# MengLing-L/distributed_plonk

Measured on AMD Instinct MI355X. Metric: constraints/sec = n / proof time (verified five-round proof, dispatcher2.rs:192-713; BN254 PLONK), higher is better.
Workload: dtype u32x8 Montgomery (256-bit Fr/Fq)

## Files before the change

### distributed_plonk_amd/csrc/msm_engine.hip

```cpp
#include <algorithm>
#include <cstring>

#include "constants.h"
#include "ec.hpp"
#include "ec_lazy.hpp"
#include "plonk_internal.hpp"

#define BASES_BAD_CURVE 1u
#define BASES_BAD_RANGE 2u
#define BASES_BAD_FLAG 4u
template <int NQ> static const FpParams<NQ>& fq_params(int curve);
template <> const FpParams<8>& fq_params<8>(int) { return BN254_FQ_PARAMS; }
template <> const FpParams<12>& fq_params<12>(int) { return BLS12_381_FQ_PARAMS; }

#ifndef MSM_SIDE_PRIO
#define MSM_SIDE_PRIO 0
#endif
#if MSM_SIDE_PRIO > 0
#define MSM_SIDE_PRIO_ENTER() __builtin_amdgcn_s_setprio(MSM_SIDE_PRIO)
#else
#define MSM_SIDE_PRIO_ENTER() ((void)0)
#endif

template <typename T> __device__ __forceinline__ T load16(const T* p) {
    static_assert(sizeof(T) % 16 == 0, "16-byte multiple");
    T r;
    const uint4* s = reinterpret_cast<const uint4*>(p);
    uint4* d = reinterpret_cast<uint4*>(&r);
#pragma unroll
    for (unsigned i = 0; i < sizeof(T) / 16; i++) d[i] = s[i];
    return r;
}
template <typename T> __device__ __forceinline__ void store16(T* p, const T& v) {
    uint4* d = reinterpret_cast<uint4*>(p);
    const uint4* s = reinterpret_cast<const uint4*>(&v);
#pragma unroll
    for (unsigned i = 0; i < sizeof(T) / 16; i++) d[i] = s[i];
}

__device__ __forceinline__ uint32_t scalar_raw_digit(const uint32_t* s, int bit0, int c) {
    const int limb = bit0 >> 5, off = bit0 & 31;
    if (limb >= 8) return 0;
    uint64_t v = s[limb];
    if (limb + 1 < 8) v |= (uint64_t)s[limb + 1] << 32;
    return (uint32_t)(v >> off) & ((1u << c) - 1);
}

__global__ void __launch_bounds__(256) msm_digits_kernel(const uint32_t* __restrict__ scalars, uint64_t n, uint64_t len, int c, int W,
                                                         uint32_t* __restrict__ dig, int scalars_mont, const FpParams<8> FR) {
    MSM_SIDE_PRIO_ENTER();
    const uint64_t i = (uint64_t)blockIdx.x * blockDim.x + threadIdx.x;
    if (i >= n) return;
    if (i >= len) {
        for (int w = 0; w < W; w++) dig[(uint64_t)w * n + i] = 0;
        return;
    }
    uint32_t s[8];
    const uint4* sp = reinterpret_cast<const uint4*>(scalars + 8 * i);
    const uint4 lo = sp[0], hi = sp[1];
    s[0] = lo.x; s[1] = lo.y; s[2] = lo.z; s[3] = lo.w; s[4] = hi.x; s[5] = hi.y; s[6] = hi.z; s[7] = hi.w;
    if (scalars_mont) {
        Fp<8> v;
#pragma unroll
        for (int k = 0; k < 8; k++) v.l[k] = s[k];
        v = fp_from_mont(v, FR);
#pragma unroll
        for (int k = 0; k < 8; k++) s[k] = v.l[k];
    }
    const uint32_t half = 1u << (c - 1);
    uint32_t carry = 0;
    for (int w = 0; w < W; w++) {
        const int bit0 = w * c, limb = bit0 >> 5, off = bit0 & 31;
        uint64_t v = 0;
#pragma unroll
        for (int k = 0; k < 8; k++) {
            if (k == limb) v |= s[k];
            if (k == limb + 1) v |= (uint64_t)s[k] << 32;
        }
        uint32_t raw = ((uint32_t)(v >> off) & ((1u << c) - 1)) + carry;
        carry = raw > half;
        const uint32_t mag = carry ? (1u << c) - raw : raw;
        dig[(uint64_t)w * n + i] = mag | (carry << 31);
    }
}

#define SORT_SLICE_LOG 14
#define SORT_SLICE (1 << SORT_SLICE_LOG)
struct SortGeom {
    uint64_t n;
    int W, cb, lp, low_bits;
    uint32_t nblk;
    uint32_t nreal;
    uint32_t idx_bits;
    uint32_t stage_cap;
};

__global__ void __launch_bounds__(256) sort_hist_kernel(const uint32_t* __restrict__ dig, SortGeom g, uint32_t* __restrict__ blk_hist) {
    MSM_SIDE_PRIO_ENTER();
    extern __shared__ uint32_t h[];
    const uint32_t np = (1u << g.lp) + 1;
    for (uint32_t k = threadIdx.x; k < np; k += blockDim.x) h[k] = 0;
    __syncthreads();
    const uint32_t w = blockIdx.y, blk = blockIdx.x;
    const uint64_t beg = (uint64_t)blk * SORT_SLICE, end = beg + SORT_SLICE < g.n ? beg + SORT_SLICE : g.n;
    const uint32_t* d = dig + (uint64_t)w * g.n;
    for (uint64_t i = beg + threadIdx.x; i < end; i += blockDim.x) {
        const uint32_t mag = d[i] & 0x7fffffffu;
        const uint32_t part = mag ? ((mag - 1) >> g.low_bits) : (np - 1);
        atomicAdd(&h[part], 1u);
    }
    __syncthreads();
    for (uint32_t k = threadIdx.x; k < np; k += blockDim.x) {
        const uint64_t pid = (k == np - 1) ? (uint64_t)g.nreal + w : ((uint64_t)w << g.lp) + k;
        blk_hist[pid * g.nblk + blk] = h[k];
    }
}

#define SCATTER_THREADS 1024
__global__ void __launch_bounds__(SCATTER_THREADS) sort_scatter_kernel(const uint32_t* __restrict__ dig, SortGeom g, const uint32_t* __restrict__ blk_off,
                                                                       uint32_t* __restrict__ tmp) {
    MSM_SIDE_PRIO_ENTER();
    extern __shared__ uint32_t sm[];
    const uint32_t np = (1u << g.lp) + 1;
    uint32_t* cnt = sm;
    uint32_t* loc = sm + np;
    uint32_t* buf = sm + 2 * np + 1;
    const uint32_t w = blockIdx.y, blk = blockIdx.x;
    for (uint32_t k = threadIdx.x; k < np; k += blockDim.x) cnt[k] = 0;
    __syncthreads();
    const uint64_t beg = (uint64_t)blk * SORT_SLICE, end = beg + SORT_SLICE < g.n ? beg + SORT_SLICE : g.n;
    const uint32_t* d = dig + (uint64_t)w * g.n;
    for (uint64_t i = beg + threadIdx.x; i < end; i += blockDim.x) {
        const uint32_t mag = d[i] & 0x7fffffffu;
        atomicAdd(&cnt[mag ? ((mag - 1) >> g.low_bits) : (np - 1)], 1u);
    }
    __syncthreads();
    __shared__ uint32_t strip[SCATTER_THREADS];
    const uint32_t per = (np + blockDim.x - 1) / blockDim.x;
    const uint32_t s0 = threadIdx.x * per < np ? threadIdx.x * per : np, s1 = s0 + per < np ? s0 + per : np;
    uint32_t acc = 0;
    for (uint32_t k = s0; k < s1; k++) acc += cnt[k];
    strip[threadIdx.x] = acc;
    __syncthreads();
    for (int dd = 1; dd < SCATTER_THREADS; dd <<= 1) {
        const uint32_t t = (int)threadIdx.x >= dd ? strip[threadIdx.x - dd] : 0;
        __syncthreads();
        strip[threadIdx.x] += t;
        __syncthreads();
    }
    uint32_t run = strip[threadIdx.x] - acc;
    for (uint32_t k = s0; k < s1; k++) { const uint32_t v = cnt[k]; loc[k] = run; cnt[k] = run; run += v; }
    if (threadIdx.x == blockDim.x - 1) loc[np] = strip[blockDim.x - 1];
    __syncthreads();
    const uint32_t low_mask = (1u << g.low_bits) - 1;
    const uint32_t ebits = (uint32_t)g.low_bits + SORT_SLICE_LOG + 1;
    const bool packed = ebits + (uint32_t)g.lp <= 32;
    for (uint64_t i = beg + threadIdx.x; i < end; i += blockDim.x) {
        const uint32_t e = d[i], mag = e & 0x7fffffffu;
        if (!mag) continue;
        const uint32_t key = mag - 1, part = key >> g.low_bits;
        const uint32_t pos = atomicAdd(&cnt[part], 1u);
        uint32_t v = ((key & low_mask) << (SORT_SLICE_LOG + 1)) | ((e >> 31) << SORT_SLICE_LOG) | (uint32_t)(i - beg);
        if (packed && g.lp) v |= part << ebits;
        buf[pos] = v;
    }
    __syncthreads();
    const uint32_t nreal_local = loc[np - 1];
    const uint32_t emask = ebits >= 32 ? 0xffffffffu : ((1u << ebits) - 1);
    for (uint32_t j = threadIdx.x; j < nreal_local; j += blockDim.x) {
        const uint32_t v = buf[j];
        uint32_t lo;
        if (packed) {
            lo = g.lp ? (v >> ebits) : 0;
        } else {
            lo = 0;
            uint32_t hi = np - 1;
            while (hi - lo > 1) { const uint32_t mid = (lo + hi) >> 1; if (loc[mid] <= j) lo = mid; else hi = mid; }
        }
        const uint64_t pid = ((uint64_t)w << g.lp) + lo;
        uint32_t out = packed ? (v & emask) : v;
        if (g.idx_bits) {
            const uint32_t in = out & (SORT_SLICE - 1), sg = (out >> SORT_SLICE_LOG) & 1u, lowb = out >> (SORT_SLICE_LOG + 1);
            out = (lowb << (g.idx_bits + 1)) | (sg << g.idx_bits) | (uint32_t)(beg + in);
        }
        tmp[blk_off[pid * g.nblk + blk] + (j - loc[lo])] = out;
    }
}

#define SIZE_BINS 256
struct SizeHist {
    uint32_t* ghist;
    uint32_t bin_shift;
    uint64_t nbuckets;
};
__device__ __forceinline__ uint32_t size_bin_of(uint32_t entries, uint32_t bin_shift) {
    const uint32_t sz = entries >> bin_shift;
    return (SIZE_BINS - 1) - (sz < SIZE_BINS - 1 ? sz : SIZE_BINS - 1);
}
__global__ void __launch_bounds__(256) sort_partition_kernel(const uint32_t* __restrict__ tmp, SortGeom g, const uint32_t* __restrict__ blk_off,
                                                             uint32_t* __restrict__ sorted, uint32_t* __restrict__ offsets, const SizeHist sz) {
    MSM_SIDE_PRIO_ENTER();
    extern __shared__ uint32_t lds[];
    __shared__ uint32_t shist[SIZE_BINS];
    if (sz.ghist) shist[threadIdx.x] = 0;
    const uint32_t nlow = 1u << g.low_bits;
    uint32_t* cnt = lds;
    uint32_t* run0 = lds + nlow;
    const uint64_t pid = blockIdx.x;
    const uint32_t* po = blk_off + pid * g.nblk;
    const uint32_t pbeg = po[0], pend = po[g.nblk];
    for (uint32_t k = threadIdx.x; k < nlow; k += blockDim.x) cnt[k] = 0;
    for (uint32_t k = threadIdx.x; k < g.nblk; k += blockDim.x) run0[k] = po[k];
    __syncthreads();
    const int sh = g.idx_bits ? (int)g.idx_bits + 1 : SORT_SLICE_LOG + 1;
    for (uint32_t j = pbeg + threadIdx.x; j < pend; j += blockDim.x) atomicAdd(&cnt[tmp[j] >> sh], 1u);
    __syncthreads();
    if (threadIdx.x == 0) {
        uint32_t run = pbeg;
        for (uint32_t k = 0; k < nlow; k++) {
            const uint32_t v = cnt[k];
            cnt[k] = run;
            run += v;
            if (sz.ghist && (pid << g.low_bits) + k < sz.nbuckets) shist[size_bin_of(v, sz.bin_shift)]++;
        }
    }
    __syncthreads();
    if (sz.ghist && shist[threadIdx.x]) atomicAdd(&sz.ghist[threadIdx.x], shist[threadIdx.x]);
    for (uint32_t k = threadIdx.x; k < nlow; k += blockDim.x) offsets[(pid << g.low_bits) + k] = cnt[k];
    if (pid == g.nreal - 1 && threadIdx.x == 0) offsets[(uint64_t)g.nreal << g.low_bits] = pend;
    __syncthreads();
    const uint32_t in_mask = SORT_SLICE - 1;
    if (g.idx_bits) {
        const uint32_t imask = (1u << g.idx_bits) - 1;
        for (uint32_t j = pbeg + threadIdx.x; j < pend; j += blockDim.x) {
            const uint32_t e = tmp[j];
            const uint32_t pos = atomicAdd(&cnt[e >> sh], 1u);
            sorted[pos] = (e & imask) | (((e >> g.idx_bits) & 1u) << 31);
        }
        return;
    }
    for (uint32_t j = pbeg + threadIdx.x; j < pend; j += blockDim.x) {
        const uint32_t e = tmp[j];
        uint32_t lo = 0, hi = g.nblk;
        while (hi - lo > 1) { const uint32_t mid = (lo + hi) >> 1; if (run0[mid] <= j) lo = mid; else hi = mid; }
        const uint32_t pos = atomicAdd(&cnt[e >> sh], 1u);
        sorted[pos] = ((lo << SORT_SLICE_LOG) + (e & in_mask)) | (((e >> SORT_SLICE_LOG) & 1u) << 31);
    }
}

#define STAGE_THREADS 1024
#define STAGE_MAX_CHUNKS 8u
__global__ void __launch_bounds__(STAGE_THREADS) sort_partition_staged_kernel(const uint32_t* __restrict__ tmp, SortGeom g, const uint32_t* __restrict__ blk_off,
                                                                              uint32_t* __restrict__ sorted, uint32_t* __restrict__ offsets, const SizeHist sz) {
    MSM_SIDE_PRIO_ENTER();
    extern __shared__ uint32_t lds[];
    __shared__ uint32_t shist[SIZE_BINS];
    if (sz.ghist && threadIdx.x < SIZE_BINS) shist[threadIdx.x] = 0;
    const uint32_t nlow = 1u << g.low_bits;
    uint32_t* cnt = lds;
    uint32_t* run0 = lds + nlow;
    uint32_t* buf = run0 + (g.idx_bits ? 0 : g.nblk);
    uint32_t* strip = buf;
    const uint64_t pid = blockIdx.x;
    const uint32_t* po = blk_off + pid * g.nblk;
    const uint32_t pbeg = po[0], pend = po[g.nblk], len = pend - pbeg;
    const int sh = g.idx_bits ? (int)g.idx_bits + 1 : SORT_SLICE_LOG + 1;
    for (uint32_t k = threadIdx.x; k < nlow; k += blockDim.x) cnt[k] = 0;
    if (!g.idx_bits)
        for (uint32_t k = threadIdx.x; k < g.nblk; k += blockDim.x) run0[k] = po[k];
    __syncthreads();
    for (uint32_t j = pbeg + threadIdx.x; j < pend; j += blockDim.x) atomicAdd(&cnt[tmp[j] >> sh], 1u);
    __syncthreads();
    const uint32_t per = (nlow + blockDim.x - 1) / blockDim.x;
    const uint32_t s0 = threadIdx.x * per < nlow ? threadIdx.x * per : nlow, s1 = s0 + per < nlow ? s0 + per : nlow;
    uint32_t acc = 0;
    for (uint32_t k = s0; k < s1; k++) acc += cnt[k];
    strip[threadIdx.x] = acc;
    __syncthreads();
    for (int dd = 1; dd < STAGE_THREADS; dd <<= 1) {
        const uint32_t t = (int)threadIdx.x >= dd ? strip[threadIdx.x - dd] : 0;
        __syncthreads();
        strip[threadIdx.x] += t;
        __syncthreads();
    }
    uint32_t run = strip[threadIdx.x] - acc;
    __syncthreads();
    for (uint32_t k = s0; k < s1; k++) {
        const uint32_t v = cnt[k];
        cnt[k] = run;
        offsets[(pid << g.low_bits) + k] = pbeg + run;
        run += v;
        if (sz.ghist && (pid << g.low_bits) + k < sz.nbuckets) atomicAdd(&shist[size_bin_of(v, sz.bin_shift)], 1u);
    }
    if (pid == g.nreal - 1 && threadIdx.x == 0) offsets[(uint64_t)g.nreal << g.low_bits] = pend;
    __syncthreads();
    if (sz.ghist && threadIdx.x < SIZE_BINS && shist[threadIdx.x]) atomicAdd(&sz.ghist[threadIdx.x], shist[threadIdx.x]);
    const uint32_t in_mask = SORT_SLICE - 1;
    const uint32_t imask = g.idx_bits ? (1u << g.idx_bits) - 1 : 0;
    const uint32_t cap = g.stage_cap;
    uint32_t nch = len <= cap ? 1u : min(nlow, (len + (cap - cap / 4) - 1) / (cap - cap / 4));
    const bool direct = nch > STAGE_MAX_CHUNKS;
    if (direct) nch = 1;
    const uint32_t bper = (nlow + nch - 1) / nch;
    for (uint32_t k0 = 0; k0 < nlow; k0 += bper) {
        const uint32_t k1 = k0 + bper < nlow ? k0 + bper : nlow;
        const uint32_t base = cnt[k0], cend = k1 < nlow ? cnt[k1] : len;
        const bool staged = !direct && cend - base <= cap;
        __syncthreads();
        for (uint32_t j = pbeg + threadIdx.x; j < pend; j += blockDim.x) {
            const uint32_t e = tmp[j], bk = e >> sh;
            if (bk < k0 || bk >= k1) continue;
            uint32_t val;
            if (g.idx_bits) {
                val = (e & imask) | (((e >> g.idx_bits) & 1u) << 31);
            } else {
                uint32_t lo = 0, hi = g.nblk;
                while (hi - lo > 1) { const uint32_t mid = (lo + hi) >> 1; if (run0[mid] <= j) lo = mid; else hi = mid; }
                val = ((lo << SORT_SLICE_LOG) + (e & in_mask)) | (((e >> SORT_SLICE_LOG) & 1u) << 31);
            }
            const uint32_t pos = atomicAdd(&cnt[bk], 1u);
            if (staged) buf[pos - base] = val; else sorted[pbeg + pos] = val;
        }
        __syncthreads();
        if (staged)
            for (uint32_t j = threadIdx.x; j < cend - base; j += blockDim.x) sorted[pbeg + base + j] = buf[j];
        __syncthreads();
    }
}

struct SetGeom {
    uint32_t cb;
    uint32_t G;
    uint32_t W1;
    uint32_t bin_shift;
    uint64_t tab_stride;
};
__device__ __forceinline__ uint64_t seg_first(const SetGeom& g, uint32_t sb, uint32_t* w0) {
    const uint32_t s = sb >> g.cb, b = sb & ((1u << g.cb) - 1u);
    const uint32_t k = s / g.G, gi = s - k * g.G;
    *w0 = gi;
    return (((uint64_t)k * g.W1 + gi) << g.cb) + b;
}
__device__ __forceinline__ uint64_t seg_step(const SetGeom& g) { return (uint64_t)g.G << g.cb; }
__device__ __forceinline__ uint32_t bucket_entries(const uint32_t* offsets, uint32_t sb, const SetGeom& g) {
    uint32_t w;
    uint64_t seg = seg_first(g, sb, &w);
    uint32_t sz = 0;
    for (; w < g.W1; w += g.G, seg += seg_step(g)) sz += offsets[seg + 1] - offsets[seg];
    return sz;
}
__device__ __forceinline__ uint32_t size_bin(const uint32_t* offsets, uint32_t sb, const SetGeom& g) {
    return size_bin_of(bucket_entries(offsets, sb, g), g.bin_shift);
}
__global__ void __launch_bounds__(256) bucket_size_hist_kernel(const uint32_t* __restrict__ offsets, uint64_t nbuckets, SetGeom g, uint32_t* __restrict__ ghist) {
    MSM_SIDE_PRIO_ENTER();
    __shared__ uint32_t h[SIZE_BINS];
    h[threadIdx.x] = 0;
    __syncthreads();
    const uint64_t b = (uint64_t)blockIdx.x * blockDim.x + threadIdx.x;
    if (b < nbuckets) atomicAdd(&h[size_bin(offsets, (uint32_t)b, g)], 1u);
    __syncthreads();
    if (h[threadIdx.x]) atomicAdd(&ghist[threadIdx.x], h[threadIdx.x]);
}
__global__ void __launch_bounds__(SIZE_BINS) bucket_size_scan_kernel(const uint32_t* __restrict__ ghist, uint32_t* __restrict__ bin_cursor) {
    MSM_SIDE_PRIO_ENTER();
    __shared__ uint32_t buf[SIZE_BINS];
    const uint32_t v = ghist[threadIdx.x];
    buf[threadIdx.x] = v;
    __syncthreads();
    for (int d = 1; d < SIZE_BINS; d <<= 1) {
        uint32_t t = (int)threadIdx.x >= d ? buf[threadIdx.x - d] : 0;
        __syncthreads();
        buf[threadIdx.x] += t;
        __syncthreads();
    }
    bin_cursor[threadIdx.x] = buf[threadIdx.x] - v;
}
__global__ void __launch_bounds__(256) bucket_size_place_kernel(const uint32_t* __restrict__ offsets, uint64_t nbuckets, SetGeom g,
                                                                uint32_t* __restrict__ bin_cursor, uint32_t* __restrict__ order, const uint32_t* __restrict__ ghist) {
    MSM_SIDE_PRIO_ENTER();
    __shared__ uint32_t h[SIZE_BINS];
    __shared__ uint32_t base[SIZE_BINS];
    __shared__ uint32_t pre[SIZE_BINS];
    h[threadIdx.x] = 0;
    uint32_t start = 0;
    if (ghist != nullptr) {
        const uint32_t v = ghist[threadIdx.x];
        pre[threadIdx.x] = v;
        __syncthreads();
        for (int d = 1; d < SIZE_BINS; d <<= 1) {
            const uint32_t t = (int)threadIdx.x >= d ? pre[threadIdx.x - d] : 0;
            __syncthreads();
            pre[threadIdx.x] += t;
            __syncthreads();
        }
        start = pre[threadIdx.x] - v;
    }
    __syncthreads();
    const uint64_t b = (uint64_t)blockIdx.x * blockDim.x + threadIdx.x;
    uint32_t bin = 0, rank = 0;
    if (b < nbuckets) { bin = size_bin(offsets, (uint32_t)b, g); rank = atomicAdd(&h[bin], 1u); }
    __syncthreads();
    if (h[threadIdx.x]) base[threadIdx.x] = start + atomicAdd(&bin_cursor[threadIdx.x], h[threadIdx.x]);
    __syncthreads();
    if (b < nbuckets) order[base[bin] + rank] = (uint32_t)b;
}

#define SCAN_ITEMS 16
#define SCAN_THREADS 256
#define SCAN_CHUNK (SCAN_ITEMS * SCAN_THREADS)

__global__ void __launch_bounds__(SCAN_THREADS) scan_block_sums_kernel(const uint32_t* __restrict__ in, uint64_t n, uint32_t* __restrict__ block_sums) {
    MSM_SIDE_PRIO_ENTER();
    __shared__ uint32_t red[SCAN_THREADS];
    const uint64_t base = (uint64_t)blockIdx.x * SCAN_CHUNK + (uint64_t)threadIdx.x * SCAN_ITEMS;
    uint32_t s = 0;
    for (int k = 0; k < SCAN_ITEMS; k++) if (base + k < n) s += in[base + k];
    red[threadIdx.x] = s;
    __syncthreads();
    for (int d = SCAN_THREADS / 2; d > 0; d >>= 1) {
        if ((int)threadIdx.x < d) red[threadIdx.x] += red[threadIdx.x + d];
        __syncthreads();
    }
    if (threadIdx.x == 0) block_sums[blockIdx.x] = red[0];
}

__global__ void __launch_bounds__(1024) scan_top_kernel(uint32_t* __restrict__ block_sums, uint64_t nblocks, uint32_t* __restrict__ total_out) {
    MSM_SIDE_PRIO_ENTER();
    __shared__ uint32_t buf[1024];
    __shared__ uint32_t carry;
    if (threadIdx.x == 0) carry = 0;
    __syncthreads();
    for (uint64_t base = 0; base < nblocks; base += 1024) {
        const uint64_t i = base + threadIdx.x;
        const uint32_t v = i < nblocks ? block_sums[i] : 0;
        buf[threadIdx.x] = v;
        __syncthreads();
        for (int d = 1; d < 1024; d <<= 1) {
            uint32_t t = (int)threadIdx.x >= d ? buf[threadIdx.x - d] : 0;
            __syncthreads();
            buf[threadIdx.x] += t;
            __syncthreads();
        }
        const uint32_t incl = buf[threadIdx.x];
        if (i < nblocks) block_sums[i] = carry + incl - v;
        __syncthreads();
        if (threadIdx.x == 1023) carry += incl;
        __syncthreads();
    }
    if (threadIdx.x == 0) *total_out = carry;
}
// ... 668 lines not shown
    }
    p.c = c; p.G = G; p.W1 = W1; p.W = W; p.cb = cb; p.Wr = Wr;
    p.nsub = nsub; p.nbuckets = nbuckets; p.heavy_thresh = heavy_thresh;
    p.max_heavy = ((uint64_t)n * W) / heavy_thresh + 1;
    p.packed = (uint32_t)g.low_bits + SORT_SLICE_LOG + 1 + (uint32_t)g.lp <= 32;
    p.nhist = ((uint64_t)g.nreal + W) * g.nblk;
    p.nscan_blocks = (p.nhist + SCAN_CHUNK - 1) / SCAN_CHUNK;
    p.nlev = 0;
    for (uint64_t cur = nb; cur > 1 && p.nlev < 15; p.nlev++) {
        p.lev_n[p.nlev] = cur;
        p.lev_k[p.nlev] = std::min<uint64_t>(REDUCE_K, cur);
        p.lev_nch[p.nlev] = cur / p.lev_k[p.nlev];
        cur = p.lev_nch[p.nlev];
    }
    p.pyr = 0;
    for (int l = 0; l < p.nlev; l++) p.pyr += (uint64_t)Wr * p.lev_nch[l];
    p.gsplit = (uint32_t)std::min<uint64_t>(32, std::max<uint64_t>(1, (p.nlev ? p.lev_nch[0] : 1) / 2048));
    p.grid_mode = ws.reduce_grid != 0 && cb >= 2;
    p.g_logL = (uint32_t)(cb + 1) / 2; p.g_logH = (uint32_t)cb - p.g_logL; p.g_nbits = p.g_logL + 1 + p.g_logH;
    p.fused_order = (ws.fused_order == 2 || (ws.fused_order == 1 && (uint64_t)n * (uint64_t)K >= ((uint64_t)1 << 23))) && sg.tab_stride == 0 && sg.G == sg.W1;
    const size_t lds_fixed = (((size_t)1 << g.low_bits) + (g.idx_bits ? 0 : g.nblk)) * 4;
    p.lds_staged = 78 * 1024;
    g.stage_cap = lds_fixed + 4096 * 4 <= p.lds_staged ? (uint32_t)((p.lds_staged - lds_fixed) / 4) : 0;
    if (ws.sort_stage_cap > 0 && g.stage_cap) g.stage_cap = std::min<uint32_t>(g.stage_cap, std::max<uint32_t>((uint32_t)ws.sort_stage_cap, STAGE_THREADS));
    p.staged = g.low_bits >= 8 && g.stage_cap >= STAGE_THREADS && !getenv("PLONK_MSM_NO_STAGED_SORT");
    p.acc_grid = (uint32_t)((nbuckets + 255) / 256);
    p.persistent = false;
    if (ws.acc_persist != 0) {
        const uint32_t pgrid = ws.acc_persist > 0 ? (uint32_t)n_cu * (uint32_t)ws.acc_persist : (uint32_t)(-ws.acc_persist);
        if (pgrid < p.acc_grid) { p.persistent = true; p.acc_grid = pgrid; }
    }
    p.sg = sg; p.g = g;
    return PLONK_OK;
}

static int device_cu_count(int* out) {
    static int cu_of_dev[64];
    int dev = 0;
    HIP_TRY(hipGetDevice(&dev));
    int n_cu = dev >= 0 && dev < 64 ? __atomic_load_n(&cu_of_dev[dev], __ATOMIC_ACQUIRE) : 0;
    if (!n_cu) {
        hipDeviceProp_t prop;
        HIP_TRY(hipGetDeviceProperties(&prop, dev));
        n_cu = std::max(prop.multiProcessorCount, 1);
        if (dev >= 0 && dev < 64) __atomic_store_n(&cu_of_dev[dev], n_cu, __ATOMIC_RELEASE);
    }
    *out = n_cu;
    return PLONK_OK;
}

static size_t msm_slice_points(const MsmWorkspace& ws) { return (size_t)1 << std::min(std::max(ws.slice_log, 8), 26); }
static int msm_group(size_t m, int K, int bits, int window_bits, const MsmTable& tab, const MsmWorkspace& ws) {
    int G_ = 1;
    const int c = plan_window(m, bits, window_bits, tab, &G_);
    const int W1 = (bits + 1 + c - 1) / c;
    const uint64_t per = (uint64_t)m * W1;
    int group = (int)std::max<uint64_t>(1, std::min<uint64_t>((uint64_t)K, (0xfffffff0ull / per)));
    if ((uint64_t)group * W1 > 65535) group = 65535 / W1;
    return std::min(group, std::min(std::max(ws.batch_max, 1), 64));
}

int msm_plan_query(int curve, size_t n, int K, const MsmWorkspace& ws, int window_bits, const MsmTable& tab, int32_t* out, int n_out) {
    if (n == 0 || K <= 0) return plonk_fail(PLONK_ERR_ARG, "msm plan: %zu points, %d vectors", n, K);
    if (!out || n_out < PLONK_MSM_PLAN_FIELDS) return plonk_fail(PLONK_ERR_ARG, "msm plan: room for %d of %d fields", out ? n_out : 0, PLONK_MSM_PLAN_FIELDS);
    const int bits = fr_params(curve).bits;
    const size_t m = std::min(msm_slice_points(ws), n);
    const int kn = std::min(msm_group(m, K, bits, window_bits, tab, ws), K);
    int n_cu = 0;
    int rc = device_cu_count(&n_cu);
    if (rc) return rc;
    MsmPlan p;
    if ((rc = msm_plan(m, kn, bits, window_bits, tab, ws, n_cu, p))) return rc;
    out[PLONK_MSM_PLAN_C] = p.c; out[PLONK_MSM_PLAN_W1] = p.W1; out[PLONK_MSM_PLAN_G] = p.G; out[PLONK_MSM_PLAN_CB] = p.cb;
    out[PLONK_MSM_PLAN_LP] = p.g.lp; out[PLONK_MSM_PLAN_LOW_BITS] = p.g.low_bits; out[PLONK_MSM_PLAN_NBLK] = (int32_t)p.g.nblk;
    out[PLONK_MSM_PLAN_IDX_BITS] = (int32_t)p.g.idx_bits; out[PLONK_MSM_PLAN_PACKED] = p.packed; out[PLONK_MSM_PLAN_STAGED] = p.staged;
    out[PLONK_MSM_PLAN_STAGE_CAP] = (int32_t)p.g.stage_cap; out[PLONK_MSM_PLAN_FUSED_ORDER] = p.fused_order; out[PLONK_MSM_PLAN_NLEV] = p.nlev;
    out[PLONK_MSM_PLAN_LAST_K] = p.nlev ? (int32_t)p.lev_k[p.nlev - 1] : 0; out[PLONK_MSM_PLAN_GSPLIT] = (int32_t)p.gsplit;
    out[PLONK_MSM_PLAN_HEAVY_THRESH] = (int32_t)std::min<uint32_t>(p.heavy_thresh, 0x7fffffffu); out[PLONK_MSM_PLAN_PERSISTENT] = p.persistent;
    out[PLONK_MSM_PLAN_GRID_MODE] = p.grid_mode; out[PLONK_MSM_PLAN_STAGE_MAX_CHUNKS] = (int32_t)STAGE_MAX_CHUNKS; out[PLONK_MSM_PLAN_STAGE_THREADS] = STAGE_THREADS;
    out[PLONK_MSM_PLAN_HEAVY_BUCKET] = (int32_t)HEAVY_BUCKET; out[PLONK_MSM_PLAN_HEAVY_SEGS] = HEAVY_SEGS; out[PLONK_MSM_PLAN_SORT_SLICE_LOG] = SORT_SLICE_LOG;
    out[PLONK_MSM_PLAN_N] = (int32_t)m; out[PLONK_MSM_PLAN_K] = kn; out[PLONK_MSM_PLAN_N_CU] = n_cu;
    out[PLONK_MSM_PLAN_ACC_GRID] = (int32_t)std::min<uint32_t>(p.acc_grid, 0x7fffffffu); out[PLONK_MSM_PLAN_BIN_SHIFT] = (int32_t)p.sg.bin_shift;
    return PLONK_OK;
}

template <int NQ>
static int msm_slice(int curve, const BaseRec<NQ>* d_bases, const uint32_t* const* d_scalars, const size_t* lens, int K, bool scalars_mont,
                     size_t n, XyzzPt<NQ>* h_result, MsmWorkspace& ws, int window_bits, const MsmTable& tab, hipStream_t stream) {
    const FpParams<NQ>& P = fq_params<NQ>(curve);
    int n_cu = 0;
    if (ws.acc_persist != 0) { const int rc_cu = device_cu_count(&n_cu); if (rc_cu) return rc_cu; }
    MsmPlan p;
    { const int rc_plan = msm_plan(n, K, fr_params(curve).bits, window_bits, tab, ws, n_cu, p); if (rc_plan) return rc_plan; }
    const int c = p.c, G = p.G, W1 = p.W1, W = p.W, cb = p.cb, Wr = p.Wr;
    const uint64_t nsub = p.nsub, nbuckets = p.nbuckets, nhist = p.nhist, nscan_blocks = p.nscan_blocks;
    const uint32_t heavy_thresh = p.heavy_thresh;
    const SetGeom sg = p.sg;
    const SortGeom g = p.g;

    size_t off = 0;
    const size_t o_dig = off; off = align_up(off + (size_t)n * W * 4, 256);
    const size_t o_tmp = off; off = align_up(off + (size_t)n * W * 4, 256);
    const size_t o_hist = off; off = align_up(off + (nhist + 1) * 4, 256);
    const size_t o_hoff = off; off = align_up(off + (nhist + 1) * 4, 256);
    const size_t o_offsets = off; off = align_up(off + (nsub + 1) * 4, 256);
    const size_t o_bsums = off; off = align_up(off + (nscan_blocks + 1) * 4, 256);
    const size_t o_sorted = off; off = align_up(off + (size_t)n * W * 4, 256);
    const size_t o_order = off; off = align_up(off + nbuckets * 4, 256);
    const size_t o_redo = off; off = align_up(off + (nbuckets + 1) * 4, 256);
    const size_t o_szh = off; off = align_up(off + 2 * SIZE_BINS * 4, 256);
    const size_t o_work = off; off = align_up(off + 4, 256);
    const uint64_t max_heavy = p.max_heavy;
    const size_t o_heavy = off; off = align_up(off + (max_heavy + 1) * 4, 256);
    typedef XyzzL<LimbGeom<NQ>::NL, LimbGeom<NQ>::B> BucketL;
    const int nlev = p.nlev;
    const uint64_t *lev_n = p.lev_n, *lev_k = p.lev_k, *lev_nch = p.lev_nch, pyr = p.pyr;
    const size_t o_buckets = off; off = align_up(off + nbuckets * sizeof(BucketL), 256);
    const size_t o_acc = off; off = align_up(off + pyr * sizeof(BucketL), 256);
    const size_t o_sarr = off; off = align_up(off + pyr * sizeof(BucketL), 256);
    const uint32_t nsplit = 1;
    const uint32_t gsplit = p.gsplit;
    const size_t o_wsum = off; off = align_up(off + (size_t)Wr * (nlev + 1) * nsplit * sizeof(XyzzPt<NQ>), 256);
    const size_t o_wpart = off; off = align_up(off + (gsplit > 1 ? (size_t)Wr * (nlev + 1) * gsplit * sizeof(BucketL) : 0), 256);
    const size_t o_hpart = off; off = align_up(off + max_heavy * HEAVY_SEGS * sizeof(BucketL), 256);
    const bool grid_mode = p.grid_mode;
    const uint32_t g_logL = p.g_logL, g_logH = p.g_logH, g_nbits = p.g_nbits;
    const size_t o_grc = off; off = align_up(off + (grid_mode ? (size_t)Wr * (((size_t)1 << g_logL) + ((size_t)1 << g_logH)) * sizeof(BucketL) : 0), 256);
    const size_t o_gbits = off; off = align_up(off + (grid_mode ? (size_t)Wr * g_nbits * sizeof(XyzzPt<NQ>) : 0), 256);
    int rc = ensure_ws(ws, off);
    if (rc) return rc;
    char* base = (char*)ws.d_buf;
    uint32_t* dig = (uint32_t*)(base + o_dig);
    uint32_t* tmp = (uint32_t*)(base + o_tmp);
    uint32_t* blk_hist = (uint32_t*)(base + o_hist);
    uint32_t* blk_off = (uint32_t*)(base + o_hoff);
    uint32_t* offsets = (uint32_t*)(base + o_offsets);
    uint32_t* bsums = (uint32_t*)(base + o_bsums);
    uint32_t* sorted = (uint32_t*)(base + o_sorted);
    uint32_t* order = (uint32_t*)(base + o_order);
    uint32_t* redo = (uint32_t*)(base + o_redo);
    uint32_t* heavy = (uint32_t*)(base + o_heavy);
    uint32_t* ghist = (uint32_t*)(base + o_szh);
    uint32_t* bin_cursor = ghist + SIZE_BINS;
    BucketL* buckets = (BucketL*)(base + o_buckets);
    BucketL* acc_arr = (BucketL*)(base + o_acc);
    BucketL* s_arr = (BucketL*)(base + o_sarr);
    XyzzPt<NQ>* wsum = (XyzzPt<NQ>*)(base + o_wsum);
    BucketL* hpart = (BucketL*)(base + o_hpart);
    BucketL* wpart = (BucketL*)(base + o_wpart);
    BucketL* grid_r = (BucketL*)(base + o_grc);
    BucketL* grid_c = grid_r + ((size_t)Wr << g_logL);
    XyzzPt<NQ>* gbits = (XyzzPt<NQ>*)(base + o_gbits);

    const size_t lds1 = ((size_t)(1u << g.lp) + 1) * 4;
    { ProfScope ps("msm_digits_kernel", stream);
    for (int k = 0; k < K; k++)
        hipLaunchKernelGGL(msm_digits_kernel, dim3((uint32_t)((n + 255) / 256)), dim3(256), 0, stream, d_scalars[k], (uint64_t)n, (uint64_t)lens[k], c, W1,
                           dig + (size_t)k * W1 * n, scalars_mont ? 1 : 0, fr_params(curve)); }
    const bool fused_order = p.fused_order;
    const SizeHist szh{fused_order ? ghist : nullptr, sg.bin_shift, (uint64_t)nbuckets};
    if (fused_order) HIP_TRY(hipMemsetAsync(ghist, 0, 2 * SIZE_BINS * 4, stream));
    { ProfScope ps("msm_sort", stream);
    hipLaunchKernelGGL(sort_hist_kernel, dim3(g.nblk, W), dim3(256), lds1, stream, dig, g, blk_hist);
    hipLaunchKernelGGL(scan_block_sums_kernel, dim3((uint32_t)nscan_blocks), dim3(SCAN_THREADS), 0, stream, blk_hist, nhist, bsums);
    hipLaunchKernelGGL(scan_top_kernel, dim3(1), dim3(1024), 0, stream, bsums, nscan_blocks, blk_off + nhist);
    hipLaunchKernelGGL(scan_apply_kernel, dim3((uint32_t)nscan_blocks), dim3(SCAN_THREADS), 0, stream, blk_hist, nhist, bsums, blk_off);
    {
        static DeviceOnce attr;
        HIP_TRY(attr.run([] { return hipFuncSetAttribute(reinterpret_cast<const void*>(&sort_scatter_kernel), hipFuncAttributeMaxDynamicSharedMemorySize, 150 * 1024); }));
    }
    hipLaunchKernelGGL(sort_scatter_kernel, dim3(g.nblk, W), dim3(SCATTER_THREADS), (2 * ((size_t)(1u << g.lp) + 1) + 1 + SORT_SLICE) * 4, stream, dig, g,
                       blk_off, tmp);
    const size_t lds_staged = p.lds_staged;
    if (p.staged) {
        static DeviceOnce attr2;
        HIP_TRY(attr2.run([] { return hipFuncSetAttribute(reinterpret_cast<const void*>(&sort_partition_staged_kernel), hipFuncAttributeMaxDynamicSharedMemorySize, 150 * 1024); }));
        hipLaunchKernelGGL(sort_partition_staged_kernel, dim3(g.nreal), dim3(STAGE_THREADS), lds_staged, stream, tmp, g, blk_off, sorted, offsets, szh);
    } else {
        hipLaunchKernelGGL(sort_partition_kernel, dim3(g.nreal), dim3(256), (((size_t)1 << g.low_bits) + g.nblk) * 4, stream, tmp, g, blk_off, sorted, offsets, szh);
    } }
    { ProfScope ps("msm_bucket_order", stream);
    HIP_TRY(hipMemsetAsync(redo, 0, 4, stream));
    HIP_TRY(hipMemsetAsync(heavy, 0, 4, stream));
    const uint32_t bgrid = (uint32_t)((nbuckets + 255) / 256);
    if (fused_order) {
        hipLaunchKernelGGL(bucket_size_place_kernel, dim3(bgrid), dim3(256), 0, stream, offsets, nbuckets, sg, bin_cursor, order, (const uint32_t*)ghist);
    } else {
        HIP_TRY(hipMemsetAsync(ghist, 0, 2 * SIZE_BINS * 4, stream));
        hipLaunchKernelGGL(bucket_size_hist_kernel, dim3(bgrid), dim3(256), 0, stream, offsets, nbuckets, sg, ghist);
        hipLaunchKernelGGL(bucket_size_scan_kernel, dim3(1), dim3(SIZE_BINS), 0, stream, ghist, bin_cursor);
        hipLaunchKernelGGL(bucket_size_place_kernel, dim3(bgrid), dim3(256), 0, stream, offsets, nbuckets, sg, bin_cursor, order, (const uint32_t*)nullptr);
    } }
    uint32_t* work = nullptr;
    const uint32_t acc_grid = p.acc_grid;
    if (p.persistent) {
        work = (uint32_t*)(base + o_work);
        HIP_TRY(hipMemsetAsync(work, 0, 4, stream));
    }
    { ProfScope ps("msm_accumulate_kernel", stream);
    if (ws.fused_y3)
        hipLaunchKernelGGL((msm_accumulate_kernel<NQ, true>), dim3(acc_grid), dim3(256), 0, stream, d_bases, sorted, offsets, order,
                           nbuckets, sg, heavy_thresh, buckets, redo, redo + 1, heavy, heavy + 1, work, fl_params<NQ>(curve));
    else
        hipLaunchKernelGGL((msm_accumulate_kernel<NQ, false>), dim3(acc_grid), dim3(256), 0, stream, d_bases, sorted, offsets, order,
                           nbuckets, sg, heavy_thresh, buckets, redo, redo + 1, heavy, heavy + 1, work, fl_params<NQ>(curve)); }
    { ProfScope ps("msm_heavy", stream);
    hipLaunchKernelGGL(msm_heavy_kernel<NQ>, dim3(128, HEAVY_SEGS), dim3(256), 256 * sizeof(BucketL), stream, d_bases, sorted, offsets, sg,
                       heavy, heavy + 1, hpart, fl_params<NQ>(curve));
    hipLaunchKernelGGL(msm_heavy_finish_kernel<NQ>, dim3(16), dim3(64), 0, stream, heavy, heavy + 1, hpart, buckets, fl_params<NQ>(curve)); }
    { ProfScope ps("msm_accumulate_redo_kernel", stream);
    hipLaunchKernelGGL(msm_accumulate_redo_kernel<NQ>, dim3(256), dim3(64), 0, stream, d_bases, sorted, offsets, sg, buckets, redo,
                       redo + 1, fl_params<NQ>(curve)); }
    if (grid_mode) {
        ProfScope ps("msm_reduce", stream);
        auto pick_seg = [&](uint32_t logY) {
            uint32_t ls = std::min<uint32_t>(logY, 6);
            while (ls > 3 && (logY - ls) < 3 && (((uint64_t)Wr << cb) >> (logY - ls + 1)) >= ((uint64_t)1 << 18)) ls--;
            return ls;
        };
        const uint32_t log_segc = pick_seg(g_logH), log_segr = pick_seg(g_logL);
        const uint32_t cwc = 256u >> log_segc, cwr = 256u >> log_segr;
        const uint32_t colblocks = (uint32_t)((((uint64_t)1 << g_logL) + cwc - 1) / cwc), rowblocks = (uint32_t)((((uint64_t)1 << g_logH) + cwr - 1) / cwr);
        hipLaunchKernelGGL(msm_grid_sums_kernel<NQ>, dim3(colblocks + rowblocks, Wr), dim3(256), 256 * sizeof(BucketL), stream, buckets, g_logL, g_logH, log_segc, log_segr,
                           colblocks, grid_r, grid_c, fl_params<NQ>(curve));
        hipLaunchKernelGGL(msm_bit_sums_kernel<NQ>, dim3(g_nbits, Wr), dim3(256), 256 * sizeof(BucketL), stream, grid_r, grid_c, g_logL, g_logH, gbits, fl_params<NQ>(curve));
    } else {
        ProfScope ps("msm_reduce", stream);
        SumJobs jobs;
        memset(&jobs, 0, sizeof jobs);
        const BucketL* in = buckets;
        uint64_t at = 0;
        for (int l = 0; l < nlev; l++) {
            const uint64_t total_chunks = (uint64_t)Wr * lev_nch[l];
            HIP_TRY(hipMemsetAsync(redo, 0, 4, stream));
            hipLaunchKernelGGL(msm_reduce_level_kernel<NQ>, dim3((uint32_t)((total_chunks + 255) / 256)), dim3(256), 0, stream, in, lev_n[l],
                               (uint32_t)lev_k[l], lev_nch[l], total_chunks, acc_arr + at, s_arr + at, redo, redo + 1, fl_params<NQ>(curve));
            hipLaunchKernelGGL(msm_reduce_level_redo_kernel<NQ>, dim3(64), dim3(64), 0, stream, in, lev_n[l], (uint32_t)lev_k[l], lev_nch[l],
                               acc_arr + at, s_arr + at, redo, redo + 1, fl_params<NQ>(curve));
            jobs.src[l] = acc_arr + at;
            jobs.count[l] = lev_nch[l];
            in = s_arr + at;
            at += total_chunks;
        }
        jobs.src[nlev] = in;
        jobs.count[nlev] = 1;
        if (gsplit > 1) {
            hipLaunchKernelGGL((msm_points_sum_kernel<NQ, true>), dim3(nlev + 1, Wr, gsplit), dim3(256), 256 * sizeof(BucketL), stream, jobs, (XyzzPt<NQ>*)nullptr,
                               (uint32_t)(nlev + 1), gsplit, fl_params<NQ>(curve), wpart);
            SumJobs fold;
            memset(&fold, 0, sizeof fold);
            for (int l = 0; l <= nlev; l++) {
                fold.src[l] = wpart + (size_t)l * gsplit;
                fold.count[l] = gsplit;
                fold.wstride[l] = (uint64_t)(nlev + 1) * gsplit;
            }
            hipLaunchKernelGGL((msm_points_sum_kernel<NQ, false>), dim3(nlev + 1, Wr, 1), dim3(256), 256 * sizeof(BucketL), stream, fold, wsum, (uint32_t)(nlev + 1), 1u,
                               fl_params<NQ>(curve), (BucketL*)nullptr);
        } else {
            hipLaunchKernelGGL((msm_points_sum_kernel<NQ, false>), dim3(nlev + 1, Wr, nsplit), dim3(256), 256 * sizeof(BucketL), stream, jobs, wsum, (uint32_t)(nlev + 1), nsplit,
                               fl_params<NQ>(curve), (BucketL*)nullptr);
        }
    }
    hipError_t e = hipGetLastError();
    if (e != hipSuccess) return plonk_fail(PLONK_ERR_HIP, "msm launch: %s", hipGetErrorString(e));

    std::vector<XyzzPt<NQ>> h(grid_mode ? (size_t)Wr * g_nbits : (size_t)Wr * (nlev + 1) * nsplit);
    HIP_TRY(hipMemcpyAsync(h.data(), grid_mode ? gbits : wsum, h.size() * sizeof(XyzzPt<NQ>), hipMemcpyDeviceToHost, stream));
    HIP_TRY(hipStreamSynchronize(stream));
    const int Wk = G;
    for (int kk = 0; kk < K; kk++) {
    XyzzPt<NQ> total = xyzz_inf<NQ>();
    for (int w = (kk + 1) * Wk - 1; w >= kk * Wk; w--) {
        if (grid_mode) {
            const XyzzPt<NQ>* tr = h.data() + (size_t)w * g_nbits;
            const XyzzPt<NQ>* tc = tr + g_logL + 1;
            XyzzPt<NQ> v = xyzz_inf<NQ>();
            for (int b = (int)(g_logL + (g_logH ? g_logH - 1 : 0)); b >= 0; b--) {
                if (!xyzz_is_inf(v)) v = xyzz_dbl(v, P);
                if (b <= (int)g_logL) v = xyzz_add(v, tr[b], P);
                if (b >= (int)g_logL && b - (int)g_logL < (int)g_logH) v = xyzz_add(v, tc[b - g_logL], P);
            }
            if (!xyzz_is_inf(total))
                for (int k = 0; k < c; k++) total = xyzz_dbl(total, P);
            total = xyzz_add(total, v, P);
            continue;
        }
        const XyzzPt<NQ>* hw = h.data() + (size_t)w * (nlev + 1) * nsplit;
        auto part = [&](int l) {
            XyzzPt<NQ> t = hw[(size_t)l * nsplit];
            for (uint32_t z = 1; z < nsplit; z++) t = xyzz_add(t, hw[(size_t)l * nsplit + z], P);
            return t;
        };
        XyzzPt<NQ> v = xyzz_inf<NQ>();
        for (int l = 0; l < nlev; l++) {
            if (!xyzz_is_inf(v))
                for (uint64_t k = lev_k[l]; k > 1; k >>= 1) v = xyzz_dbl(v, P);
            v = xyzz_add(v, part(l), P);
        }
        v = xyzz_add(v, part(nlev), P);
        if (!xyzz_is_inf(total))
            for (int k = 0; k < c; k++) total = xyzz_dbl(total, P);
        total = xyzz_add(total, v, P);
    }
    h_result[kk] = total;
    }
    return PLONK_OK;
}


template <int NQ>
static int msm_run_t(int curve, const void* d_bases, const uint32_t* const* d_scalars, const size_t* lens, int K, bool scalars_mont, size_t n, uint32_t* h_out_jac,
                     MsmWorkspace& ws, int window_bits, const MsmTable& tab, hipStream_t stream) {
    const FpParams<NQ>& P = fq_params<NQ>(curve);
    std::vector<XyzzPt<NQ>> total((size_t)K, xyzz_inf<NQ>());
    const size_t SLICE = msm_slice_points(ws);
    for (size_t s = 0; s < n; s += SLICE) {
// ... 64 lines not shown
```

Baseline: 21.69 million.

## Fuse scalar digit extraction with sort histogram and keep scatter entries in registers

Merges the per-vector digit kernel and the per-window histogram kernel into one launch over all scalar vectors. Each block decomposes scalars into signed digits and builds LDS histograms for groups of windows in the same pass, avoiding a separate re-read of the digit array for the first window group. The scatter and staged partition kernels now hold their input entries in registers between the count pass and the placement pass, so they no longer read global memory twice. These kernels also get occupancy hints through launch bounds. The trade-offs are higher register pressure from the 18-entry keep array, a cap of 64 vectors per launch, and extra digit re-reads for window groups after the first when LDS cannot hold every histogram at once.

```diff
diff --git a/distributed_plonk_amd/csrc/msm_engine.hip b/distributed_plonk_amd/csrc/msm_engine.hip
--- a/distributed_plonk_amd/csrc/msm_engine.hip
+++ b/distributed_plonk_amd/csrc/msm_engine.hip
@@ -44,44 +44,6 @@
     uint64_t v = s[limb];
     if (limb + 1 < 8) v |= (uint64_t)s[limb + 1] << 32;
     return (uint32_t)(v >> off) & ((1u << c) - 1);
-}
-
-__global__ void __launch_bounds__(256) msm_digits_kernel(const uint32_t* __restrict__ scalars, uint64_t n, uint64_t len, int c, int W,
-                                                         uint32_t* __restrict__ dig, int scalars_mont, const FpParams<8> FR) {
-    MSM_SIDE_PRIO_ENTER();
-    const uint64_t i = (uint64_t)blockIdx.x * blockDim.x + threadIdx.x;
-    if (i >= n) return;
-    if (i >= len) {
-        for (int w = 0; w < W; w++) dig[(uint64_t)w * n + i] = 0;
-        return;
-    }
-    uint32_t s[8];
-    const uint4* sp = reinterpret_cast<const uint4*>(scalars + 8 * i);
-    const uint4 lo = sp[0], hi = sp[1];
-    s[0] = lo.x; s[1] = lo.y; s[2] = lo.z; s[3] = lo.w; s[4] = hi.x; s[5] = hi.y; s[6] = hi.z; s[7] = hi.w;
-    if (scalars_mont) {
-        Fp<8> v;
-#pragma unroll
-        for (int k = 0; k < 8; k++) v.l[k] = s[k];
-        v = fp_from_mont(v, FR);
-#pragma unroll
-        for (int k = 0; k < 8; k++) s[k] = v.l[k];
-    }
-    const uint32_t half = 1u << (c - 1);
-    uint32_t carry = 0;
-    for (int w = 0; w < W; w++) {
-        const int bit0 = w * c, limb = bit0 >> 5, off = bit0 & 31;
-        uint64_t v = 0;
-#pragma unroll
-        for (int k = 0; k < 8; k++) {
-            if (k == limb) v |= s[k];
-            if (k == limb + 1) v |= (uint64_t)s[k] << 32;
-        }
-        uint32_t raw = ((uint32_t)(v >> off) & ((1u << c) - 1)) + carry;
-        carry = raw > half;
-        const uint32_t mag = carry ? (1u << c) - raw : raw;
-        dig[(uint64_t)w * n + i] = mag | (carry << 31);
-    }
 }
 
 #define SORT_SLICE_LOG 14
@@ -95,29 +57,86 @@
     uint32_t stage_cap;
 };
 
-__global__ void __launch_bounds__(256) sort_hist_kernel(const uint32_t* __restrict__ dig, SortGeom g, uint32_t* __restrict__ blk_hist) {
+#define MSM_MAX_GROUP 64
+#define DIGHIST_THREADS 1024
+#define DIGHIST_LDS_WORDS (78 * 256)
+struct ScalarVecs {
+    const uint32_t* ptr[MSM_MAX_GROUP];
+    uint64_t len[MSM_MAX_GROUP];
+};
+__global__ void __launch_bounds__(DIGHIST_THREADS, 8) sort_digits_hist_kernel(const ScalarVecs sv, SortGeom g, int c, int W1, int wgroup, uint32_t* dig,
+                                                                           uint32_t* __restrict__ blk_hist, int scalars_mont, const FpParams<8> FR) {
     MSM_SIDE_PRIO_ENTER();
     extern __shared__ uint32_t h[];
     const uint32_t np = (1u << g.lp) + 1;
-    for (uint32_t k = threadIdx.x; k < np; k += blockDim.x) h[k] = 0;
-    __syncthreads();
-    const uint32_t w = blockIdx.y, blk = blockIdx.x;
+    const uint32_t kv = blockIdx.y, blk = blockIdx.x;
+    const uint32_t* __restrict__ scalars = sv.ptr[kv];
+    const uint64_t len = sv.len[kv];
     const uint64_t beg = (uint64_t)blk * SORT_SLICE, end = beg + SORT_SLICE < g.n ? beg + SORT_SLICE : g.n;
-    const uint32_t* d = dig + (uint64_t)w * g.n;
-    for (uint64_t i = beg + threadIdx.x; i < end; i += blockDim.x) {
-        const uint32_t mag = d[i] & 0x7fffffffu;
-        const uint32_t part = mag ? ((mag - 1) >> g.low_bits) : (np - 1);
-        atomicAdd(&h[part], 1u);
-    }
-    __syncthreads();
-    for (uint32_t k = threadIdx.x; k < np; k += blockDim.x) {
-        const uint64_t pid = (k == np - 1) ? (uint64_t)g.nreal + w : ((uint64_t)w << g.lp) + k;
-        blk_hist[pid * g.nblk + blk] = h[k];
+    uint32_t* d = dig + (uint64_t)kv * W1 * g.n;
+    const uint32_t half = 1u << (c - 1);
+    for (int w0 = 0; w0 < W1; w0 += wgroup) {
+        const int w1 = w0 + wgroup < W1 ? w0 + wgroup : W1;
+        const uint32_t nh = (uint32_t)(w1 - w0) * np;
+        for (uint32_t k = threadIdx.x; k < nh; k += blockDim.x) h[k] = 0;
+        __syncthreads();
+        for (uint64_t i = beg + threadIdx.x; i < end; i += blockDim.x) {
+            if (w0 > 0) {
+                for (int w = w0; w < w1; w++) {
+                    const uint32_t mag = d[(uint64_t)w * g.n + i] & 0x7fffffffu;
+                    atomicAdd(&h[(uint32_t)(w - w0) * np + (mag ? ((mag - 1) >> g.low_bits) : (np - 1))], 1u);
+                }
+                continue;
+            }
+            if (i >= len) {
+                for (int w = 0; w < W1; w++) {
+                    d[(uint64_t)w * g.n + i] = 0;
+                    if (w < w1) atomicAdd(&h[(uint32_t)w * np + (np - 1)], 1u);
+                }
+                continue;
+            }
+            uint32_t s[8];
+            const uint4* sp = reinterpret_cast<const uint4*>(scalars + 8 * i);
+            const uint4 lo = sp[0], hi = sp[1];
+            s[0] = lo.x; s[1] = lo.y; s[2] = lo.z; s[3] = lo.w; s[4] = hi.x; s[5] = hi.y; s[6] = hi.z; s[7] = hi.w;
+            if (scalars_mont) {
+                Fp<8> v;
+#pragma unroll
+                for (int k = 0; k < 8; k++) v.l[k] = s[k];
+                v = fp_from_mont(v, FR);
+#pragma unroll
+                for (int k = 0; k < 8; k++) s[k] = v.l[k];
+            }
+            uint32_t carry = 0;
+            for (int w = 0; w < W1; w++) {
+                const int bit0 = w * c, limb = bit0 >> 5, off = bit0 & 31;
+                uint64_t v = 0;
+#pragma unroll
+                for (int k = 0; k < 8; k++) {
+                    if (k == limb) v |= s[k];
+                    if (k == limb + 1) v |= (uint64_t)s[k] << 32;
+                }
+                const uint32_t raw = ((uint32_t)(v >> off) & ((1u << c) - 1)) + carry;
+                carry = raw > half;
+                const uint32_t mag = carry ? (1u << c) - raw : raw;
+                d[(uint64_t)w * g.n + i] = mag | (carry << 31);
+                if (w < w1) atomicAdd(&h[(uint32_t)w * np + (mag ? ((mag - 1) >> g.low_bits) : (np - 1))], 1u);
+            }
+        }
+        __syncthreads();
+        for (uint32_t k = threadIdx.x; k < nh; k += blockDim.x) {
+            const uint32_t wl = k / np, kk = k - wl * np;
+            const uint64_t w = (uint64_t)kv * W1 + w0 + wl;
+            const uint64_t pid = (kk == np - 1) ? (uint64_t)g.nreal + w : (w << g.lp) + kk;
+            blk_hist[pid * g.nblk + blk] = h[k];
+        }
+        __syncthreads();
     }
 }
 
 #define SCATTER_THREADS 1024
-__global__ void __launch_bounds__(SCATTER_THREADS) sort_scatter_kernel(const uint32_t* __restrict__ dig, SortGeom g, const uint32_t* __restrict__ blk_off,
+#define SCATTER_PER (SORT_SLICE / SCATTER_THREADS)
+__global__ void __launch_bounds__(SCATTER_THREADS, 8) sort_scatter_kernel(const uint32_t* __restrict__ dig, SortGeom g, const uint32_t* __restrict__ blk_off,
                                                                        uint32_t* __restrict__ tmp) {
     MSM_SIDE_PRIO_ENTER();
     extern __shared__ uint32_t sm[];
@@ -130,9 +149,16 @@
     __syncthreads();
     const uint64_t beg = (uint64_t)blk * SORT_SLICE, end = beg + SORT_SLICE < g.n ? beg + SORT_SLICE : g.n;
     const uint32_t* d = dig + (uint64_t)w * g.n;
-    for (uint64_t i = beg + threadIdx.x; i < end; i += blockDim.x) {
-        const uint32_t mag = d[i] & 0x7fffffffu;
-        atomicAdd(&cnt[mag ? ((mag - 1) >> g.low_bits) : (np - 1)], 1u);
+    uint32_t e[SCATTER_PER];
+#pragma unroll
+    for (int r = 0; r < SCATTER_PER; r++) {
+        const uint64_t i = beg + threadIdx.x + (uint32_t)r * SCATTER_THREADS;
+        e[r] = i < end ? d[i] : 0u;
+    }
+#pragma unroll
+    for (int r = 0; r < SCATTER_PER; r++) {
+        const uint32_t mag = e[r] & 0x7fffffffu;
+        if (mag) atomicAdd(&cnt[(mag - 1) >> g.low_bits], 1u);
     }
     __syncthreads();
     __shared__ uint32_t strip[SCATTER_THREADS];
@@ -155,12 +181,13 @@
     const uint32_t low_mask = (1u << g.low_bits) - 1;
     const uint32_t ebits = (uint32_t)g.low_bits + SORT_SLICE_LOG + 1;
     const bool packed = ebits + (uint32_t)g.lp <= 32;
-    for (uint64_t i = beg + threadIdx.x; i < end; i += blockDim.x) {
-        const uint32_t e = d[i], mag = e & 0x7fffffffu;
+#pragma unroll
+    for (int r = 0; r < SCATTER_PER; r++) {
+        const uint32_t mag = e[r] & 0x7fffffffu;
         if (!mag) continue;
         const uint32_t key = mag - 1, part = key >> g.low_bits;
         const uint32_t pos = atomicAdd(&cnt[part], 1u);
-        uint32_t v = ((key & low_mask) << (SORT_SLICE_LOG + 1)) | ((e >> 31) << SORT_SLICE_LOG) | (uint32_t)(i - beg);
+        uint32_t v = ((key & low_mask) << (SORT_SLICE_LOG + 1)) | ((e[r] >> 31) << SORT_SLICE_LOG) | (threadIdx.x + (uint32_t)r * SCATTER_THREADS);
         if (packed && g.lp) v |= part << ebits;
         buf[pos] = v;
     }
@@ -250,7 +277,8 @@
 
 #define STAGE_THREADS 1024
 #define STAGE_MAX_CHUNKS 8u
-__global__ void __launch_bounds__(STAGE_THREADS) sort_partition_staged_kernel(const uint32_t* __restrict__ tmp, SortGeom g, const uint32_t* __restrict__ blk_off,
+#define STAGE_KEEP 18
+__global__ void __launch_bounds__(STAGE_THREADS, 8) sort_partition_staged_kernel(const uint32_t* __restrict__ tmp, SortGeom g, const uint32_t* __restrict__ blk_off,
                                                                               uint32_t* __restrict__ sorted, uint32_t* __restrict__ offsets, const SizeHist sz) {
     MSM_SIDE_PRIO_ENTER();
     extern __shared__ uint32_t lds[];
@@ -269,7 +297,18 @@
     if (!g.idx_bits)
         for (uint32_t k = threadIdx.x; k < g.nblk; k += blockDim.x) run0[k] = po[k];
     __syncthreads();
-    for (uint32_t j = pbeg + threadIdx.x; j < pend; j += blockDim.x) atomicAdd(&cnt[tmp[j] >> sh], 1u);
+    const bool keep = len <= g.stage_cap && len <= (uint32_t)STAGE_KEEP * STAGE_THREADS;
+    uint32_t ent[STAGE_KEEP];
+    if (keep) {
+#pragma unroll
+        for (int r = 0; r < STAGE_KEEP; r++) {
+            const uint32_t j = pbeg + threadIdx.x + (uint32_t)r * STAGE_THREADS;
+            ent[r] = j < pend ? tmp[j] : 0u;
+            if (j < pend) atomicAdd(&cnt[ent[r] >> sh], 1u);
+        }
+    } else {
+        for (uint32_t j = pbeg + threadIdx.x; j < pend; j += blockDim.x) atomicAdd(&cnt[tmp[j] >> sh], 1u);
+    }
     __syncthreads();
     const uint32_t per = (nlow + blockDim.x - 1) / blockDim.x;
     const uint32_t s0 = threadIdx.x * per < nlow ? threadIdx.x * per : nlow, s1 = s0 + per < nlow ? s0 + per : nlow;
@@ -297,6 +336,26 @@
     if (sz.ghist && threadIdx.x < SIZE_BINS && shist[threadIdx.x]) atomicAdd(&sz.ghist[threadIdx.x], shist[threadIdx.x]);
     const uint32_t in_mask = SORT_SLICE - 1;
     const uint32_t imask = g.idx_bits ? (1u << g.idx_bits) - 1 : 0;
+    if (keep) {
+#pragma unroll
+        for (int r = 0; r < STAGE_KEEP; r++) {
+            const uint32_t j = pbeg + threadIdx.x + (uint32_t)r * STAGE_THREADS;
+            if (j >= pend) continue;
+            const uint32_t e = ent[r];
+            uint32_t val;
+            if (g.idx_bits) {
+                val = (e & imask) | (((e >> g.idx_bits) & 1u) << 31);
+            } else {
+                uint32_t lo = 0, hi = g.nblk;
+                while (hi - lo > 1) { const uint32_t mid = (lo + hi) >> 1; if (run0[mid] <= j) lo = mid; else hi = mid; }
+                val = ((lo << SORT_SLICE_LOG) + (e & in_mask)) | (((e >> SORT_SLICE_LOG) & 1u) << 31);
+            }
+            buf[atomicAdd(&cnt[e >> sh], 1u)] = val;
+        }
+        __syncthreads();
+        for (uint32_t j = threadIdx.x; j < len; j += blockDim.x) sorted[pbeg + j] = buf[j];
+        return;
+    }
     const uint32_t cap = g.stage_cap;
     uint32_t nch = len <= cap ? 1u : min(nlow, (len + (cap - cap / 4) - 1) / (cap - cap / 4));
     const bool direct = nch > STAGE_MAX_CHUNKS;
@@ -1271,16 +1330,21 @@
     BucketL* grid_c = grid_r + ((size_t)Wr << g_logL);
     XyzzPt<NQ>* gbits = (XyzzPt<NQ>*)(base + o_gbits);
 
-    const size_t lds1 = ((size_t)(1u << g.lp) + 1) * 4;
-    { ProfScope ps("msm_digits_kernel", stream);
-    for (int k = 0; k < K; k++)
-        hipLaunchKernelGGL(msm_digits_kernel, dim3((uint32_t)((n + 255) / 256)), dim3(256), 0, stream, d_scalars[k], (uint64_t)n, (uint64_t)lens[k], c, W1,
-                           dig + (size_t)k * W1 * n, scalars_mont ? 1 : 0, fr_params(curve)); }
     const bool fused_order = p.fused_order;
     const SizeHist szh{fused_order ? ghist : nullptr, sg.bin_shift, (uint64_t)nbuckets};
     if (fused_order) HIP_TRY(hipMemsetAsync(ghist, 0, 2 * SIZE_BINS * 4, stream));
     { ProfScope ps("msm_sort", stream);
-    hipLaunchKernelGGL(sort_hist_kernel, dim3(g.nblk, W), dim3(256), lds1, stream, dig, g, blk_hist);
+    {
+        if (K > MSM_MAX_GROUP) return plonk_fail(PLONK_ERR_ARG, "msm: %d vectors in one launch set", K);
+        ScalarVecs sv;
+        for (int k = 0; k < MSM_MAX_GROUP; k++) { sv.ptr[k] = k < K ? d_scalars[k] : nullptr; sv.len[k] = k < K ? (uint64_t)lens[k] : 0; }
+        const uint32_t np = (1u << g.lp) + 1;
+        const int wgroup = std::min<int>(W1, std::max<int>(1, (int)(DIGHIST_LDS_WORDS / np)));
+        static DeviceOnce attr0;
+        HIP_TRY(attr0.run([] { return hipFuncSetAttribute(reinterpret_cast<const void*>(&sort_digits_hist_kernel), hipFuncAttributeMaxDynamicSharedMemorySize, 150 * 1024); }));
+        hipLaunchKernelGGL(sort_digits_hist_kernel, dim3(g.nblk, (uint32_t)K), dim3(DIGHIST_THREADS), (size_t)wgroup * np * 4, stream, sv, g, c, W1, wgroup, dig,
+                           blk_hist, scalars_mont ? 1 : 0, fr_params(curve));
+    }
     hipLaunchKernelGGL(scan_block_sums_kernel, dim3((uint32_t)nscan_blocks), dim3(SCAN_THREADS), 0, stream, blk_hist, nhist, bsums);
     hipLaunchKernelGGL(scan_top_kernel, dim3(1), dim3(1024), 0, stream, bsums, nscan_blocks, blk_off + nhist);
     hipLaunchKernelGGL(scan_apply_kernel, dim3((uint32_t)nscan_blocks), dim3(SCAN_THREADS), 0, stream, blk_hist, nhist, bsums, blk_off);
```

After: 21.97 million (median of 6 runs). 1.3% higher.
